# dmlc/difacto

Hardware: AMD Instinct MI355X
Metric: examples/sec (FM SGD worker step, Criteo-shape, V_dim=64) (higher is better)
Workload: dtype f32

## Files before the change

difacto_amd/capi.py:

```python
import ctypes as C
import os

import numpy as np

_HERE = os.path.dirname(os.path.abspath(__file__))
LIB_PATH = os.environ.get("DIFACTO_HIP_LIB") or os.path.join(_HERE, "libdifacto_hip.so")

FEA_COUNT, WEIGHT, GRADIENT = 1, 2, 3
INIT_REFRAND, INIT_HASH = 0, 1
U64MAX = 2 ** 64 - 1

SYMBOLS = [
    "dfh_last_error", "dfh_updater_param_default", "dfh_ctx_create", "dfh_ctx_destroy", "dfh_ctx_sync",
    "dfh_ctx_stream", "dfh_ctx_device", "dfh_reverse_bytes", "dfh_encode_fea_grp_id", "dfh_table_create",
    "dfh_table_destroy", "dfh_table_size", "dfh_table_param", "dfh_table_bytes", "dfh_pull", "dfh_push",
    "dfh_table_export", "dfh_table_import", "dfh_fm_predict", "dfh_fm_calcgrad", "dfh_loss_evaluate",
    "dfh_auc_times_n", "dfh_batch_create", "dfh_batch_destroy", "dfh_batch_load_host", "dfh_batch_load_device",
    "dfh_localize", "dfh_batch_load_localized_host", "dfh_batch_get_localized", "dfh_batch_shape", "dfh_sgd_step",
    "dfh_batch_progress", "dfh_batch_get_pred", "dfh_row_stride", "dfh_shard_pull", "dfh_shard_push_count",
    "dfh_shard_push_grad", "dfh_batch_forward", "dfh_batch_backward", "dfh_batch_device_keys", "dfh_malloc",
    "dfh_free", "dfh_memcpy_h2d", "dfh_memcpy_d2h", "dfh_ctx_set_timing", "dfh_ctx_get_timing", "dfh_kernel_name",
    "dfh_table_warm_start", "dfh_ctx_set_pipeline", "dfh_batch_lookup", "dfh_localize_lookup", "dfh_rowbuf_create", "dfh_rowbuf_destroy", "dfh_rowbuf_load_host", "dfh_batch_gather_rows", "dfh_batch_set_option", "dfh_batch_key_ranges", "dfh_batch_attach_device",
    "dfh_batch_key_ranges_device", "dfh_shard_resolve", "dfh_shard_pull_resolved", "dfh_shard_push_count_resolved",
    "dfh_shard_push_grad_resolved", "dfh_table_check", "dfh_ctx_set_timing_mask", "dfh_table_save", "dfh_table_load", "dfh_shard_resolve_multi", "dfh_shard_push_count_multi",
    "dfh_shard_push_grad_multi", "dfh_shard_count_pull_multi", "dfh_shard_push_grad_listed", "dfh_shard_release", "dfh_ctx_set_option", "dfh_table_set_has_aux", "dfh_table_has_aux",
    "dfh_comm_unique_id", "dfh_comm_create_rccl", "dfh_comm_create_callback", "dfh_comm_destroy", "dfh_comm_rank", "dfh_comm_world",
    "dfh_comm_allreduce_sum", "dfh_shard_create", "dfh_shard_destroy", "dfh_shard_owned_range", "dfh_shard_step", "dfh_shard_prefetch_counts",
    "dfh_shard_pull_host", "dfh_shard_push_host", "dfh_comm_allgather", "dfh_shard_balanced_splits", "dfh_shard_set_exchange", "dfh_shard_set_timing", "dfh_shard_get_timing",
    "dfh_comm_stats", "dfh_comm_info", "dfh_comm_selfcheck", "dfh_comm_wire_probe", "dfh_table_capacity", "dfh_batch_prepare_rows", "dfh_rowbuf_load_host_slices",
    "dfh_rowbuf_set_labels", "dfh_batch_prepare_cached", "dfh_batch_get_rows",
    "dfh_batch_create_many", "dfh_shard_multi_words", "dfh_shard_reserve", "dfh_comm_create_loopback", "dfh_comm_loopback_feed", "dfh_comm_loopback_wire", "dfh_comm_loopback_wire_time",
    "dfh_vec_inner_multi", "dfh_vec_combine", "dfh_vec_line_step", "dfh_lbfgs_create", "dfh_lbfgs_destroy", "dfh_lbfgs_add_chunk",
    "dfh_lbfgs_init_model", "dfh_lbfgs_shape", "dfh_lbfgs_get_model", "dfh_lbfgs_set_weights", "dfh_lbfgs_calc_grad",
    "dfh_lbfgs_prepare_direction", "dfh_lbfgs_calc_direction", "dfh_lbfgs_line_search", "dfh_lbfgs_evaluate", "dfh_lbfgs_create_sharded",
    "dfh_lbfgs_owned_range", "dfh_lbfgs_set_model", "dfh_bcd_set_model",
    "dfh_bcd_create", "dfh_bcd_destroy", "dfh_bcd_add_chunk", "dfh_bcd_build", "dfh_bcd_shape", "dfh_bcd_block_info",
    "dfh_bcd_epoch", "dfh_bcd_step", "dfh_bcd_get_model", "dfh_bcd_get_pred", "dfh_batch_split_entries",
    "dfh_bcd_create_sharded",
    "dfh_textchunk_create", "dfh_textchunk_destroy", "dfh_textchunk_parse_criteo", "dfh_textchunk_rows", "dfh_textchunk_ids",
    "dfh_rowbuf_load_slices",
]
XCHG_COUNTS, XCHG_KEYS, XCHG_CNT, XCHG_ROWS, XCHG_GRADS, XCHG_OTHER = range(6)
SHARD_STAGES = ("counts", "L", "K", "R", "RW", "F", "G", "P")
K_COUNT = 8
K_LOCALIZE, K_LOOKUP, K_FORWARD, K_BACKWARD, K_PULL, K_PUSH, K_MISC, K_AUC = range(8)


class UpdaterParam(C.Structure):
    _fields_ = [("l1", C.c_float), ("l2", C.c_float), ("V_l2", C.c_float), ("lr", C.c_float),
                ("lr_beta", C.c_float), ("V_lr", C.c_float), ("V_lr_beta", C.c_float),
                ("V_init_scale", C.c_float), ("V_dim", C.c_int), ("V_threshold", C.c_int),
                ("seed", C.c_uint), ("init_mode", C.c_int)]
# ... 30 lines not shown
            "%s is missing: build it with `python -m difacto_amd.build` (hipcc --offload-arch=gfx950). "
            "There is no CPU fallback." % LIB_PATH)
    if os.environ.get("DIFACTO_NO_TORCH_PRELOAD") != "1":
        try:
            import torch
        except ImportError:
            pass
    L = C.CDLL(LIB_PATH)
    vp, sz, i32, u64, f32 = C.c_void_p, C.c_size_t, C.c_int, C.c_uint64, C.c_float
    PP = C.POINTER
    L.dfh_last_error.restype = C.c_char_p
    L.dfh_updater_param_default.argtypes = [PP(UpdaterParam), i32]
    L.dfh_ctx_create.argtypes = [i32, vp, PP(vp)]
    L.dfh_ctx_destroy.argtypes = [vp]
    L.dfh_ctx_sync.argtypes = [vp]
    L.dfh_ctx_stream.restype = vp
    L.dfh_ctx_stream.argtypes = [vp]
    L.dfh_ctx_device.argtypes = [vp]
    L.dfh_reverse_bytes.restype = u64
    L.dfh_reverse_bytes.argtypes = [u64]
    L.dfh_encode_fea_grp_id.restype = u64
    L.dfh_encode_fea_grp_id.argtypes = [u64, i32, i32]
    L.dfh_table_create.argtypes = [vp, PP(UpdaterParam), u64, PP(vp)]
    L.dfh_table_destroy.argtypes = [vp]
    L.dfh_table_size.argtypes = [vp, PP(u64)]
    L.dfh_table_param.argtypes = [vp, PP(UpdaterParam)]
    L.dfh_table_capacity.argtypes = [vp, PP(u64), PP(u64)]
    L.dfh_table_bytes.restype = u64
    L.dfh_table_bytes.argtypes = [vp]
    L.dfh_pull.argtypes = [vp, vp, sz, vp, PP(sz), vp, PP(sz)]
    L.dfh_push.argtypes = [vp, vp, sz, i32, vp, sz, vp, sz]
    L.dfh_table_export.argtypes = [vp, u64, vp, vp, vp, vp, PP(u64)]
    L.dfh_table_import.argtypes = [vp, u64, vp, vp, vp, vp]
    L.dfh_fm_predict.argtypes = [vp, i32, sz, vp, vp, vp, vp, sz, vp, vp, sz, vp]
    L.dfh_fm_calcgrad.argtypes = [vp, i32, sz, vp, vp, vp, vp, vp, sz, vp, vp, sz, vp, vp]
    L.dfh_loss_evaluate.argtypes = [vp, vp, vp, sz, PP(f32)]
    L.dfh_auc_times_n.argtypes = [vp, vp, vp, sz, PP(f32)]
    L.dfh_batch_create.argtypes = [vp, sz, sz, PP(vp)]
    L.dfh_batch_destroy.argtypes = [vp]
    L.dfh_batch_create_many.argtypes = [vp, i32, sz, sz, PP(vp)]
    L.dfh_batch_split_entries.argtypes = [vp, vp]
    L.dfh_batch_load_host.argtypes = [vp, sz, vp, vp, vp, vp]
    L.dfh_batch_load_device.argtypes = [vp, sz, sz, vp, vp, vp, vp]
    L.dfh_batch_attach_device.argtypes = [vp, sz, sz, vp, vp, vp, vp]
    L.dfh_localize.argtypes = [vp, u64]
    L.dfh_batch_load_localized_host.argtypes = [vp, sz, vp, vp, vp, vp, vp, vp, sz]
    L.dfh_batch_get_localized.argtypes = [vp, PP(sz), vp, vp, vp]
    L.dfh_batch_shape.argtypes = [vp, PP(sz), PP(sz), PP(sz)]
    L.dfh_sgd_step.argtypes = [vp, vp, i32, i32]
    L.dfh_batch_progress.argtypes = [vp, PP(Progress), i32]
    L.dfh_batch_get_pred.argtypes = [vp, vp]
    L.dfh_row_stride.restype = sz
    L.dfh_row_stride.argtypes = [i32]
    L.dfh_shard_pull.argtypes = [vp, vp, sz, vp]
    L.dfh_shard_push_count.argtypes = [vp, vp, sz, vp]
    L.dfh_shard_push_grad.argtypes = [vp, vp, sz, vp]
# ... 147 lines not shown
class Context:

    def __init__(self, device=0, stream=None):
        self.h = C.c_void_p()
        _ck(lib().dfh_ctx_create(device, _dp(stream), C.byref(self.h)))

    def sync(self):
        _ck(lib().dfh_ctx_sync(self.h))

    def set_pipeline(self, on=True):
        _ck(lib().dfh_ctx_set_pipeline(self.h, int(on)))

    def set_option(self, name, value):
        _ck(lib().dfh_ctx_set_option(self.h, name.encode(), int(value)))

    def set_timing(self, on=True):
        _ck(lib().dfh_ctx_set_timing(self.h, 1 if on else 0))

    def set_timing_mask(self, mask):
        _ck(lib().dfh_ctx_set_timing_mask(self.h, mask))

    def get_timing(self, reset=True):
        ms = np.zeros(K_COUNT, np.float64)
        calls = np.zeros(K_COUNT, np.uint64)
        _ck(lib().dfh_ctx_get_timing(self.h, 1 if reset else 0, _p(ms), _p(calls)))
        return {lib().dfh_kernel_name(i).decode(): (float(ms[i]), int(calls[i])) for i in range(K_COUNT)}

    @property
    def stream(self):
        return lib().dfh_ctx_stream(self.h)
# ... 376 lines not shown
    def progress(self, reset=True):
        p = Progress()
        _ck(lib().dfh_batch_progress(self.h, C.byref(p), 1 if reset else 0))
        return p

    def pred(self):
        nrows, _, _ = self.shape(want_U=False)
        out = np.zeros(nrows, np.float32)
        _ck(lib().dfh_batch_get_pred(self.h, _p(out)))
        return out

    def split_entries(self):
        n = C.c_uint32(0)
        _ck(lib().dfh_batch_split_entries(self.h, C.byref(n)))
        return int(n.value)

    def forward(self, V_dim, d_rows):
        _ck(lib().dfh_batch_forward(self.h, V_dim, _dp(d_rows)))

    def backward(self, V_dim, d_rows, d_grads):
        _ck(lib().dfh_batch_backward(self.h, V_dim, _dp(d_rows), _dp(d_grads)))

    def key_ranges(self, nparts):
        out = np.zeros(nparts + 1, np.uint32)
        _ck(lib().dfh_batch_key_ranges(self.h, nparts, _p(out)))
        return out

    def device_keys(self):
        a, b, u = C.c_void_p(), C.c_void_p(), C.c_size_t(0)
        _ck(lib().dfh_batch_device_keys(self.h, C.byref(a), C.byref(b), C.byref(u)))
# ... 389 lines not shown
```

difacto_amd/csrc/dfh_api.hip:

```cpp
#include <algorithm>
#include <chrono>
#include <cstring>
#include <mutex>
#include <new>
#include <thread>

#include <hip/hip_ext.h>
#include <rocprim/rocprim.hpp>

#include "dfh_kernels.hip"
#include "dfh_localize.hip"
#include "dfh_update.hip"
#include "dfh_riders.hip"

using namespace dfh;

namespace dfh {
static thread_local std::string g_err;
void set_error(const std::string& msg) { g_err = msg; }
}

struct dfh_ctx {
  int device = 0;
  hipStream_t stream = nullptr;
  bool own_stream = false;
  std::vector<hipStream_t> preps;
  std::vector<hipStream_t> extra;
  hipStream_t parse = nullptr;
  std::mutex parse_mu;
  unsigned nprep = 0;
  unsigned next_prep = 0;
  bool pipeline = false;
  void* scratch = nullptr;
  size_t scratch_bytes = 0;
  int num_cu = 256;
  int fwd_depth = 5;
  int fwd_blocks = 0;
  int bwd_small_blocks = 2048;
  int upd_kernel = 1;
  int upd_hot_blocks = 512, upd_mid_blocks = 512, upd_few_blocks = 1024, upd_single_blocks = 4096;
  int upd_interleave = 0;
  int owner_per_key = 0;
  int upd_split = 1;
  int auc_in_update = 1;
  int shard_mixed_update = 1;
  int grow_initial_rows = 1 << 20;
  int event_flags = 1;
  int prep_priority = -1;
  int single_queue = 0;
  int rider_slot[4] = {2, 0, 1, 2};
  int rider_alone[4] = {0, 0, 0, 0};
  int rider_period[3] = {1, 1, 1};
  int rider_start[3] = {0, 0, 0};
  std::vector<dfh_batch*> pend;
  std::thread warm;
// ... 101 lines not shown
  uint32_t* d_split_ticket = nullptr;
  float* d_split_part = nullptr;
  size_t split_cap = 0;
  int split_sel = 0, split_last = 0;
  bool split_listing = false;
  uint32_t seg_nb = 0;
  uint2* d_uw = nullptr;
  uint32_t *d_urow = nullptr, *d_need = nullptr, *d_rank = nullptr, *d_total = nullptr;
  float *d_pred = nullptr, *d_slope = nullptr, *d_xv = nullptr;
  size_t xv_floats = 0;
  static constexpr size_t kProgDoubles = 2 * PROG_SLOTS + 64;
  double* d_prog = nullptr;
  float nrows_seen = 0;
  hipEvent_t ev_ready = nullptr, ev_free = nullptr;
  bool ready_pending = false, free_pending = false;
  hipStream_t prep = nullptr;
  bool compute_auc = false;
  uint32_t *d_auc_keys = nullptr, *d_auc_skeys = nullptr, *d_auc_lab = nullptr, *d_auc_slab = nullptr;
  uint32_t* d_auc_part = nullptr;
  uint32_t auc_pending_n = 0;
  bool force_radix = false;
  bool force_sort_fallback = false;
  dfh_table* looked_up = nullptr;
  struct GatherSeg { struct dfh_rowbuf* rb; size_t at, n; };
  std::vector<GatherSeg> gsegs;
  GatherSrc gsrc{};
  bool gather_pending = false, gather_fusable = false, gather_any_value = false, loc_fuse_gather = false;
  const uint32_t *g_rows = nullptr, *g_off = nullptr;
  const float* g_lab = nullptr;
  LocView loc_v{};
// ... 4 lines not shown
};

namespace dfh {
namespace chunks {
inline hipError_t reset_prog(dfh_batch* b, hipStream_t s);
}
}

namespace {
int flush_pending(dfh_batch* b);
void pend_remove(dfh_ctx* c, dfh_batch* b);
inline hipStream_t prep_of(const dfh_batch* b) {
  const dfh_ctx* c = b->ctx;
  return (c->pipeline && b->prep) ? b->prep : c->stream;
}
void phase_begin(dfh_batch* b) {
  dfh_ctx* c = b->ctx;
  if (b->pend_stage < RID_STAGES) (void)flush_pending(b);
  hipStream_t next = c->pipeline ? c->preps[c->next_prep++ % c->nprep] : nullptr;
  if (next && b->prep && next != b->prep && b->ready_pending) {
    (void)hipStreamWaitEvent(next, b->ev_ready, 0);
  }
  b->prep = next;
}
int prep_begin(dfh_batch* b) {
  dfh_ctx* c = b->ctx;
  if (c->pipeline && !b->prep) phase_begin(b);
  if (c->pipeline && b->free_pending) {
    DFH_HIP(hipStreamWaitEvent(prep_of(b), b->ev_free, 0));
    b->free_pending = false;
  }
  return DFH_OK;
}
int prep_end(dfh_batch* b) {
  dfh_ctx* c = b->ctx;
  if (c->pipeline && !b->defer_ready) {
    DFH_HIP(hipEventRecord(b->ev_ready, prep_of(b)));
    b->ready_pending = true;
  }
  return DFH_OK;
}
int main_begin(dfh_batch* b) {
  dfh_ctx* c = b->ctx;
  if (b->pend_stage < RID_STAGES) {
    int rc = flush_pending(b);
    if (rc) return rc;
  }
  if (b->ready_pending) {
    DFH_HIP(hipStreamWaitEvent(c->stream, b->ev_ready, 0));
    b->ready_pending = false;
  }
  return DFH_OK;
}
int main_end(dfh_batch* b) {
  dfh_ctx* c = b->ctx;
  if (b->split_listing) {
    b->split_listing = false;
    b->split_last = b->split_sel;
    b->split_sel ^= 1;
  }
  if (c->pipeline) {
    DFH_HIP(hipEventRecord(b->ev_free, c->stream));
    b->free_pending = true;
  }
  return DFH_OK;
}
int sync_all(dfh_ctx* c) {
  for (hipStream_t p : c->preps) DFH_HIP(hipStreamSynchronize(p));
  for (hipStream_t p : c->extra) DFH_HIP(hipStreamSynchronize(p));
  DFH_HIP(hipStreamSynchronize(c->stream));
  return DFH_OK;
}
inline bool split_listed(const dfh_ctx* c, const dfh_batch* b, int is_train) { return b && is_train && c->upd_kernel && c->upd_split; }
inline uint32_t* split_counter(const dfh_batch* b) { return b->d_U + 2 + b->split_sel; }
inline SplitOut split_out(const dfh_ctx* c, dfh_batch* b, int is_train, uint32_t u_base) {
  if (!split_listed(c, b, is_train)) return SplitOut{nullptr, nullptr, 0u, 0u};
  b->split_listing = true;
  return SplitOut{b->d_split_ent, split_counter(b), u_base, (uint32_t)b->split_cap};
}
}

namespace {

inline int grid_for_threads(size_t n, const dfh_ctx* c) {
  size_t b = (n + 255) / 256;
  size_t cap = (size_t)c->num_cu * 8;
  return (int)std::max<size_t>(1, std::min(b, cap));
}
inline int grid_for_waves(size_t nwaves, const dfh_ctx* c) {
  size_t b = (nwaves + 3) / 4;
  size_t cap = (size_t)c->num_cu * 8;
  return (int)std::max<size_t>(1, std::min(b, cap));
}

int ensure_scratch(dfh_ctx* c, size_t bytes) {
  if (bytes <= c->scratch_bytes) return DFH_OK;
  if (c->scratch) {
    DFH_HIP(hipStreamSynchronize(c->stream));
    DFH_HIP(hipFree(c->scratch));
    c->scratch = nullptr;
    c->scratch_bytes = 0;
  }
// ... 491 lines not shown

inline int count_mode(const dfh_ctx* c, int is_train, int push_cnt) { return push_cnt ? ((is_train && c->upd_kernel) ? 2 : 1) : 0; }

struct StepExtras {
  uint32_t* need = nullptr;
  bool pre = false;
  bool riders = false;
  bool spans = false;
};

int step_lookup(dfh_table* t, dfh_batch* b, int is_train, int push_cnt, uint32_t lo, const uint32_t* d_n, size_t n, const StepExtras& x,
                const float* rrows = nullptr, size_t U = 0, hipEvent_t rows_in = nullptr) {
  dfh_ctx* c = t->ctx;
  hipStream_t s = c->stream;
  const float* cnt = b->has_cnt ? b->d_feacnt + lo : (const float*)nullptr;
  const int mode = count_mode(c, is_train, push_cnt), gl = grid_for_threads(n, c);
  const uint32_t n_static = d_n ? 0u : (uint32_t)n;
  static const bool gap_trace = getenv("DFH_GAP_TRACE") != nullptr;
  const bool ride = x.spans && gap_trace && ((c->timing >> DFH_K_LOOKUP) & 1u);
  TimeScope ts(c, (x.spans && !ride) ? DFH_K_LOOKUP : DFH_K_COUNT);
  const SplitOut so = split_out(c, b, is_train, lo);
  RiderSet rs;
  rs.n = 0;
  if (x.riders) collect_riders(c, 0, true, ((uint32_t)gl + 7u) / 8u, &rs);
  if (rrows) {
    DFH_HIP(hipStreamWaitEvent(s, rows_in, 0));
    const UwRemote m{rrows, dfh_row_stride(t->v.k), b->d_U, lo, lo + (uint32_t)n, b->d_uw, b->d_col_ptr, split_out(c, b, is_train, 0u), t->v.err};
    hipLaunchKernelGGL(k_lookup_uw_remote, dim3(grid_for_threads(U, c)), dim3(256), 0, s, t->v, b->d_feaids + lo, n_static, b->d_urow + lo,
                       cnt, b->d_col_ptr + lo, mode, b->d_uw + lo, auc_pending(b), m, so);
  } else if (rs.n) {
    hipLaunchKernelGGL(k_lookup_riders, dim3((((unsigned)gl + 7u) / 8u + rs.ngroups) * 8u), dim3(256), rider_smem(rs), s, t->v,
                       b->d_feaids + lo, d_n, n_static, b->d_urow + lo, cnt, b->d_col_ptr + lo, mode, x.need, x.pre ? 1 : 0, b->d_uw + lo,
                       auc_pending(b), so, (uint32_t)gl, rs);
  } else {
    launch_span(c, ride, DFH_K_LOOKUP, 1, k_lookup_step, dim3(gl), dim3(256), 0, s, t->v, b->d_feaids + lo, d_n, n_static, b->d_urow + lo,
                cnt, b->d_col_ptr + lo, mode, x.need, x.pre ? 1 : 0, b->d_uw + lo, auc_pending(b), so);
  }
  b->auc_pending_n = 0;
  DFH_HIP(hipGetLastError());
  return DFH_OK;
}

struct StepRemote {
// ... 193 lines not shown
  } else if (n == "grow_initial_rows") {
    DFH_ARG(value >= 16 && value <= (1 << 28), "grow_initial_rows must be in [16, 2^28]");
    c->grow_initial_rows = value;
  } else if (n == "auc_in_update") {
    DFH_ARG(value == 0 || value == 1, "auc_in_update must be 0 (k_auc_pairs as its own launch) or 1 (a role of k_update_fused)");
    c->auc_in_update = value;
  } else if (n == "shard_mixed_update") {
    DFH_ARG(value == 0 || value == 1, "shard_mixed_update must be 0 or 1");
    c->shard_mixed_update = value;
  } else if (n == "owner_per_key") {
    DFH_ARG(value == 0 || value == 1, "owner_per_key must be 0 (count push, Pull, gradient push per received entry) or 1 (per distinct key)");
    c->owner_per_key = value;
  } else if (n == "upd_split") {
    DFH_ARG(value == 0 || value == 1, "upd_split must be 0 (one block per hot key, whatever its length) or 1 (a block per part of 1 024 occurrences)");
    c->upd_split = value;
  } else if (n == "upd_interleave") {
    DFH_ARG(value >= 0 && value <= 64, "upd_interleave must be in [0, 64]");
    c->upd_interleave = value;
  } else if (n == "event_flags") {
    DFH_ARG(value == 0 || value == 1, "event_flags must be 0 (default events) or 1 (no system-scope fence); set before batches are created");
    c->event_flags = value;
  } else if (n == "single_queue") {
    DFH_ARG(value == 0 || value == 1, "single_queue must be 0 (preparation streams) or 1 (the Localizer's stages ride in the step's launches)");
    if (value != c->single_queue) {
      for (dfh_batch* p : std::vector<dfh_batch*>(c->pend)) {
        int rcf = flush_pending(p);
        if (rcf) return rcf;
      }
      int rcs = sync_all(c);
      if (rcs) return rcs;
// ... 11 lines not shown
    c->rider_alone[st] = (value >> 2) & 1;
  } else if (n == "rider_start_lookup" || n == "rider_start_forward" || n == "rider_start_update") {
    DFH_ARG(value >= 0 && value <= 100, "rider_start_*: per cent of the carrier's own blocks dispatched before the first rider group");
    c->rider_start[n == "rider_start_lookup" ? 0 : n == "rider_start_forward" ? 1 : 2] = value;
  } else if (n == "rider_period_lookup" || n == "rider_period_forward" || n == "rider_period_update") {
    DFH_ARG(value >= 1 && value <= 4096, "rider_period_*: one group of 8 rider blocks every n groups (1: riders first)");
    c->rider_period[n == "rider_period_lookup" ? 0 : n == "rider_period_forward" ? 1 : 2] = value;
  } else if (n == "prep_priority") {
    DFH_ARG(value >= -1 && value <= 1, "prep_priority must be -1 (lowest), 0 (default) or 1 (highest)");
    DFH_ARG(c->preps.empty(), "prep_priority must be set before dfh_ctx_set_pipeline creates the streams");
    c->prep_priority = value;
  } else {
    set_error("dfh_ctx_set_option: unknown option " + n);
    return DFH_ERR_ARG;
  }
  return DFH_OK;
}
void* dfh_ctx_stream(dfh_ctx* c) { return c ? c->stream : nullptr; }
int dfh_ctx_device(dfh_ctx* c) { return c ? c->device : -1; }

int dfh_ctx_set_timing(dfh_ctx* c, int enable) {
  DFH_ARG(c, "ctx is NULL");
  c->timing = enable ? ~0u : 0u;
  return DFH_OK;
}

int dfh_ctx_set_timing_mask(dfh_ctx* c, uint32_t mask) {
  DFH_ARG(c, "ctx is NULL");
  c->timing = mask;
  return DFH_OK;
// ... 1419 lines not shown
  } else {
    hipLaunchKernelGGL(k_rdx_keys, dim3(g), dim3(256), 0, s, b->d_raw, N, max_index, b->d_keys, b->d_pos);
    size_t tb = b->temp_bytes;
    DFH_HIP(rocprim::radix_sort_pairs(b->d_temp, tb, b->d_keys, b->d_skeys, b->d_pos, b->d_spos, (size_t)N, 0, 64, s));
    hipLaunchKernelGGL(k_rdx_heads, dim3(g), dim3(256), 0, s, b->d_skeys, N, b->d_head);
    tb = b->temp_bytes;
    DFH_HIP(rocprim::inclusive_scan(b->d_temp, tb, b->d_head, b->d_uid, (size_t)N, rocprim::plus<uint32_t>(), s));
    hipLaunchKernelGGL(k_rdx_emit, dim3(g), dim3(256), 0, s, b->d_skeys, b->d_spos, b->d_head, b->d_uid, N, (uint32_t)b->nrows,
                       b->d_offset, b->has_value ? b->d_value : (const float*)nullptr, b->d_feaids, b->d_col_ptr, b->d_index,
                       b->d_s_row, b->d_s_val, b->d_U);
    hipLaunchKernelGGL(k_seg_lists_reset, dim3(1), dim3(64), 0, s, b->d_mid, b->d_hot, b->d_few, b->d_U + 2);
    hipLaunchKernelGGL(k_seg_lists, dim3((unsigned)std::max<size_t>(1, std::min<size_t>((N + 1023) / 1024, 256))), dim3(1024), 0, s,
                       b->d_col_ptr, b->d_U, b->d_mid, b->d_hot, b->d_few, b->d_mid_ent, b->d_hot_ent, b->d_few_ent);
    b->seg_nb = 1;
    if (probe)
      hipLaunchKernelGGL(k_lookup, dim3(grid_for_threads(b->nnz, c)), dim3(256), 0, s, probe->v, b->d_feaids, b->d_U, 0u, b->d_urow,
                         (const float*)nullptr, b->d_col_ptr, 0, (uint32_t*)nullptr, 0, (uint2*)nullptr, AucFin{nullptr, 0u, nullptr});
  }
  delete tsp;
  DFH_HIP(hipGetLastError());
  b->localized = true;
  b->has_cnt = false;
  if (probe) b->looked_up = probe;
  return prep_end(b);
}
}


int dfh_localize(dfh_batch* b, uint64_t max_index) {
  DFH_ARG(b && b->nrows > 0, "dfh_localize: no batch loaded");
  DFH_ARG(max_index != 0, "max_index must be nonzero");
// ... 35 lines not shown
    set_error("dfh_batch_lookup: batch is not localized");
    return DFH_ERR_STATE;
  }
  dfh_ctx* c = b->ctx;
  if (b->nnz == 0) return DFH_OK;
  if (b->nnz <= kSmallBatchPairs) return DFH_OK;
  if (c->single_queue) return DFH_OK;
  DFH_HIP(hipSetDevice(c->device));
  int rc = table_reserve(t, b->nnz);
  if (rc) return rc;
  rc = prep_begin(b);
  if (rc) return rc;
  {
    hipStream_t ps = prep_of(b);
    TimeScope ts(c, DFH_K_LOOKUP, ps);
    hipLaunchKernelGGL(k_lookup, dim3(grid_for_threads(b->nnz, c)), dim3(256), 0, ps, t->v, b->d_feaids, b->d_U, 0u,
                       b->d_urow, (const float*)nullptr, b->d_col_ptr, 0, (uint32_t*)nullptr, 0, (uint2*)nullptr, AucFin{nullptr, 0u, nullptr});
  }
  DFH_HIP(hipGetLastError());
  b->looked_up = t;
  return prep_end(b);
}

int dfh_batch_load_localized_host(dfh_batch* b, size_t nrows, const size_t* offset, const uint32_t* index, const float* value,
                                  const float* label, const uint64_t* feaids, const float* feacnt, size_t U) {
  DFH_ARG(b && offset && label && feaids, "dfh_batch_load_localized_host: NULL argument");
  DFH_ARG(nrows >= 1 && nrows <= b->max_rows, "nrows out of range");
  std::vector<uint32_t> off32;
  int rc = to_u32_offsets(offset, nrows, &off32);
  if (rc) return rc;
  const size_t base = offset[0], nnz = off32[nrows];
// ... 196 lines not shown
  if (is_train && refrand) {
    rc = refrand_flush(t, b->d_feaids, b->d_U, Nb, b->d_urow, b->d_need, b->d_rank, b->d_total);
    if (rc) return rc;
  }
  return main_end(b);
}

int dfh_batch_split_entries(dfh_batch* b, uint32_t* n) {
  DFH_ARG(b && n, "dfh_batch_split_entries: NULL argument");
  dfh_ctx* c = b->ctx;
  DFH_HIP(hipSetDevice(c->device));
  if (b->pend_stage < RID_STAGES) {
    int rc = flush_pending(b);
    if (rc) return rc;
  }
  if (b->ready_pending) DFH_HIP(hipStreamWaitEvent(c->stream, b->ev_ready, 0));
  DFH_HIP(hipMemcpyAsync(n, b->d_U + 2 + b->split_last, sizeof(uint32_t), hipMemcpyDeviceToHost, c->stream));
  DFH_HIP(hipStreamSynchronize(c->stream));
  return DFH_OK;
}

int dfh_batch_forward(dfh_batch* b, int V_dim, const float* d_rows) {
  DFH_ARG(b && b->localized && d_rows, "dfh_batch_forward: bad argument");
  const int kp = (V_dim + 3) / 4 * 4;
  int rc = ensure_xv(b, kp);
  if (rc) return rc;
  b->nrows_seen += (float)b->nrows;
  rc = main_begin(b);
  if (rc) return rc;
  rc = launch_forward(b, packed_src(d_rows, V_dim), V_dim, kp);
  if (rc) return rc;
  return main_end(b);
}
// ... 99 lines not shown
```

difacto_amd/csrc/dfh_feed.hip:

```cpp
struct dfh_rowbuf {
  dfh_ctx* ctx = nullptr;
  size_t max_rows = 0, max_nnz = 0, nrows = 0, nnz = 0;
  uint32_t* d_off = nullptr;
  uint64_t* d_idx = nullptr;
  float* d_val = nullptr;
  float* d_lab = nullptr;
  bool has_value = false, has_labels = false;
  hipStream_t up = nullptr;
  hipEvent_t ev_loaded = nullptr;
  struct Used { hipStream_t stream; hipEvent_t ev; bool pending; };
  std::mutex mu;
  std::vector<Used> used;
  std::vector<hipStream_t> seen_loaded;
  double t_prof[3] = {0, 0, 0};
  uint64_t n_prof = 0, bytes_prof = 0;
  std::vector<uint32_t> off32;
};

namespace {
int localize_impl(dfh_batch* b, uint64_t max_index, dfh_table* probe);

struct PrepLaps {
  double* acc;
  bool on;
// ... 303 lines not shown
  gs.dst_off = b->d_offset;
  gs.dst_lab = b->d_label;
  batch_loaded(b, nrows, in.nnz, in.any_value);
  return DFH_OK;
}

int queue_described(dfh_table* t, dfh_batch* b, const DescribedIn& in, uint64_t max_index, PrepLaps& laps) {
  dfh_ctx* c = b->ctx;
  int rc = describe(b, in);
  if (rc) return rc;
  laps.lap(3);
  b->defer_ready = true;
  rc = localize_impl(b, max_index, nullptr);
  laps.lap(4);
  if (!rc && in.nnz > kSmallBatchPairs && !c->single_queue) {
    hipLaunchKernelGGL(k_lookup, dim3(grid_for_threads(b->nnz, c)), dim3(256), 0, prep_of(b), t->v, b->d_feaids, b->d_U, 0u, b->d_urow,
                       (const float*)nullptr, b->d_col_ptr, 0, (uint32_t*)nullptr, 0, (uint2*)nullptr, AucFin{nullptr, 0u, nullptr});
    if (hipGetLastError() != hipSuccess) rc = DFH_ERR_HIP;
    b->looked_up = t;
  }
  b->defer_ready = false;
  if (rc) return rc;
  rc = prep_end(b);
  laps.lap(5);
  if (laps.on) ++b->n_prof;
  return rc;
}
}

extern "C" {

// ... 224 lines not shown
```

difacto_amd/csrc/dfh_kernels.hip:

```cpp
#include "dfh_internal.h"

namespace dfh {

__device__ __forceinline__ int lane_id() { return threadIdx.x & 63; }

__device__ __forceinline__ float wave_sum(float v) {
#pragma unroll
  for (int o = 32; o > 0; o >>= 1) v += __shfl_xor(v, o, 64);
  return v;
}

template <int L>
__device__ __forceinline__ float cross_group_sum(float v) {
#pragma unroll
  for (int o = L; o < 64; o <<= 1) v += __shfl_xor(v, o, 64);
  return v;
}
template <int L>
__device__ __forceinline__ float in_group_sum(float v) {
#pragma unroll
  for (int o = L >> 1; o > 0; o >>= 1) v += __shfl_xor(v, o, 64);
  return v;
}

// ... 378 lines not shown
  uint32_t u_base;
  uint32_t cap;
};
__device__ __forceinline__ uint32_t* split_other(uint32_t* n) { return reinterpret_cast<uint32_t*>(reinterpret_cast<uintptr_t>(n) ^ 4u); }
__device__ __forceinline__ void lookup_split(const SplitOut& so, uint32_t* err, uint32_t u, uint32_t beg, uint32_t end) {
  if (!(DFH_HOT_SPLIT_BUILD & 1) || !so.ent || end - beg <= HOT_SPLIT_MIN) return;
  const uint32_t nparts = (end - beg + HOT_SPLIT - 1u) / HOT_SPLIT;
  const uint32_t base = atomicAdd(so.n, nparts);
  if (base + nparts > so.cap) {
    atomicOr(err, 16u);
    return;
  }
  for (uint32_t p = 0; p < nparts; ++p)
    so.ent[base + p] = make_uint4(u + so.u_base, beg + p * HOT_SPLIT, min(beg + (p + 1u) * HOT_SPLIT, end), (p << 16) | nparts);
}

template <bool SPLIT = true>
__device__ __forceinline__ void lookup_body(const TableView& t, const uint64_t* __restrict__ keys, const uint32_t* __restrict__ d_n,
                         uint32_t n_static, uint32_t* __restrict__ urow, const float* __restrict__ cnt,
                         const uint32_t* __restrict__ col_ptr, int push_cnt, uint32_t* __restrict__ need_init,
                         int rows_known, uint2* __restrict__ uw, AucFin fin, const uint32_t bid, const uint32_t nblk,
                         const SplitOut so = SplitOut{nullptr, nullptr, 0u, 0u}) {
  if (fin.n && bid == 0) auc_finalize_block(fin);
  if (SPLIT && so.n && bid == 0 && threadIdx.x == 0) *split_other(so.n) = 0u;
  uint32_t n = d_n ? *d_n : n_static;
  __shared__ uint32_t ins_sh[8];
  for (uint32_t u0 = bid * blockDim.x; u0 < n; u0 += nblk * blockDim.x) {
    const uint32_t u = u0 + threadIdx.x;
    const bool active = u < n;
    uint64_t key = active ? keys[u] : 0ull;
// ... 1781 lines not shown
```

difacto_amd/csrc/dfh_shard.hip:

```cpp
#ifndef DFH_SHARD_HIP_
#define DFH_SHARD_HIP_
#include <dlfcn.h>
#include <link.h>

#include <chrono>
#include <deque>
#include <optional>
#include <thread>

namespace dfh {

struct RcclId { char internal[128]; };
struct RcclApi {
  void* lib = nullptr;
  int (*GetUniqueId)(RcclId*) = nullptr;
  int (*CommInitRank)(void**, int, RcclId, int) = nullptr;
  int (*CommDestroy)(void*) = nullptr;
  const char* (*GetErrorString)(int) = nullptr;
  int (*Send)(const void*, size_t, int, int, void*, hipStream_t) = nullptr;
  int (*Recv)(void*, size_t, int, int, void*, hipStream_t) = nullptr;
  int (*GroupStart)() = nullptr;
  int (*GroupEnd)() = nullptr;
  int (*GetVersion)(int*) = nullptr;
  std::string path;
// ... 1066 lines not shown
int shard_step_overlap(dfh_shard* s, dfh_batch* b, int is_train, int push_cnt, int* any_active) {
  dfh_comm* c = s->c;
  dfh_ctx* ctx = s->t->ctx;
  DFH_HIP(hipSetDevice(ctx->device));
  hipStream_t st = ctx->stream, cs = s->cs;
  int rc;
  if (s->timing) ++s->stage_steps;
  static const bool trace = getenv("DFH_SHARD_TRACE") != nullptr;
  Flight& cur = s->fl[s->cur];
  if (trace)
    fprintf(stderr, "[shard %d] step %llu: b=%p cur{slot %d described %d pulled %d b=%p} armed %d next_b=%p\n", c->rank,
            (unsigned long long)s->steps, (void*)b, s->cur, (int)cur.described, (int)cur.pulled, (void*)cur.b, (int)s->next_armed,
            (void*)s->next_b);
  if (!(cur.described && cur.b == b)) {
    DFH_ARG(!cur.described || !cur.pulled, "dfh_shard_step: the batch differs from the one announced to dfh_shard_prefetch_counts");
    if (b && b->ready_pending) DFH_HIP(hipStreamWaitEvent(cs, b->ev_ready, 0));
    {
      StageScope ts(s, DFH_SHARD_STAGE_COUNTS, cs);
      rc = queue_counts(s, b, cs);
      if (rc) return rc;
    }
    DFH_HIP(hipStreamSynchronize(cs));
    flight_sizes(s, cur, b, s->cur);
  }
  if (any_active) *any_active = cur.active != 0 ? 1 : 0;
  ++s->steps;
  if (b) b->nrows_seen += (float)b->nrows;
  const bool look = s->next_armed;
  dfh_batch* nb = look ? s->next_b : nullptr;
  s->next_armed = false;
  Flight& nxt = s->fl[s->cur ^ 1];
  nxt = Flight();
  if (cur.active == 0) {
    cur = Flight();
    return b ? main_end(b) : DFH_OK;
  }
  auto keys_out = [&](Flight& f) {
    const int q = f.slot;
    hipEvent_t ready = f.b && f.b->ready_pending ? f.b->ev_ready : nullptr;
    hipEvent_t freed = s->p_pending[q] ? s->ev_p[q] : nullptr;
    s->p_pending[q] = false;
    return flight_K(s, f, push_cnt, cs, ready, freed, s->ev_k[q]);
  };
  auto rows_back = [&](Flight& f) {
    const int q = f.slot;
    int r = flight_R(s, f, push_cnt, s->ev_k[q], s->ev_r[q]);
    if (!r) r = flight_RW(s, f, cs, s->ev_r[q], s->ev_rw[q]);
    f.pulled = r == DFH_OK;
    return r;
  };
  rc = flight_bufs(s, cur);
  if (rc) return rc;
  if (b) {
    rc = main_begin(b);
    if (rc) return rc;
  }
  const int q = cur.slot;
  const bool uw_folded = cur.any_own && cur.pulled && cur.any_remote && b != nullptr;
  if ((rc = flight_L(s, cur, is_train, push_cnt, uw_folded ? s->ev_rw[q] : nullptr))) return rc;
  if (!cur.pulled) {
    if ((rc = keys_out(cur)) || (rc = rows_back(cur))) return rc;
  }
  if (look) {
    if (nb && nb->ready_pending) DFH_HIP(hipStreamWaitEvent(cs, nb->ev_ready, 0));
    StageScope ts(s, DFH_SHARD_STAGE_COUNTS, cs);
    rc = queue_counts(s, nb, cs);
    if (rc) return rc;
    DFH_HIP(hipEventRecord(s->cnt_ev, cs));
  }
  if ((rc = flight_F(s, cur, is_train, push_cnt, uw_folded, uw_folded ? nullptr : s->ev_rw[q], s->ev_f))) return rc;
  bool ahead = false;
  if (look) {
    DFH_HIP(hipEventSynchronize(s->cnt_ev));
    flight_sizes(s, nxt, nb, s->cur ^ 1);
    ahead = nxt.active != 0;
    if (trace)
      fprintf(stderr, "[shard %d]   next: active %zu U %zu nrecv %zu own [%u, %u) -> ahead %d\n", c->rank, nxt.active, nxt.U, nxt.nrecv,
              nxt.own_lo, nxt.own_hi, (int)ahead);
    if (ahead) {
// ... 318 lines not shown
```

include/difacto_hip.h:

```cpp
#ifndef DIFACTO_HIP_H_
#define DIFACTO_HIP_H_
#include <stddef.h>
#include <stdint.h>

#ifdef __cplusplus
extern "C" {
#endif

enum {
  DFH_OK = 0,
  DFH_ERR_ARG = 1,
  DFH_ERR_HIP = 2,
  DFH_ERR_CAPACITY = 3,
  DFH_ERR_STATE = 4
};

enum { DFH_FEA_COUNT = 1, DFH_WEIGHT = 2, DFH_GRADIENT = 3 };

enum {
  DFH_INIT_REFRAND = 0,
  DFH_INIT_HASH = 1
};

typedef struct {
// ... 13 lines not shown
typedef struct dfh_ctx dfh_ctx;
typedef struct dfh_table dfh_table;
typedef struct dfh_batch dfh_batch;

const char* dfh_last_error(void);
void dfh_updater_param_default(dfh_updater_param* p, int V_dim);

int dfh_ctx_create(int device, void* stream, dfh_ctx** out);
int dfh_ctx_destroy(dfh_ctx* ctx);
int dfh_ctx_sync(dfh_ctx* ctx);
void* dfh_ctx_stream(dfh_ctx* ctx);
int dfh_ctx_device(dfh_ctx* ctx);

int dfh_ctx_set_pipeline(dfh_ctx* ctx, int enable);
int dfh_ctx_set_option(dfh_ctx* ctx, const char* name, int value);

enum {
  DFH_K_LOCALIZE = 0, DFH_K_LOOKUP, DFH_K_FORWARD, DFH_K_BACKWARD, DFH_K_PULL, DFH_K_PUSH, DFH_K_MISC, DFH_K_AUC, DFH_K_COUNT
};
int dfh_ctx_set_timing(dfh_ctx* ctx, int enable);
int dfh_ctx_set_timing_mask(dfh_ctx* ctx, uint32_t mask);
int dfh_ctx_get_timing(dfh_ctx* ctx, int reset, double* total_ms, uint64_t* calls);
const char* dfh_kernel_name(int id);

uint64_t dfh_reverse_bytes(uint64_t x);
uint64_t dfh_encode_fea_grp_id(uint64_t x, int gid, int nbits);

int dfh_table_create(dfh_ctx* ctx, const dfh_updater_param* p, uint64_t capacity_rows, dfh_table** out);
int dfh_table_capacity(dfh_table* t, uint64_t* capacity_rows, uint64_t* grows);
int dfh_table_destroy(dfh_table* t);
// ... 72 lines not shown
int dfh_rowbuf_set_labels(dfh_rowbuf* rb, size_t nrows, const float* label);
int dfh_batch_prepare_cached(dfh_table* t, dfh_batch* b, size_t nrows, int nseg, dfh_rowbuf* const* bufs, const uint32_t* const* rows,
                             const size_t* seg_rows, uint64_t max_index);

int dfh_batch_load_localized_host(dfh_batch* b, size_t nrows, const size_t* offset, const uint32_t* index,
                                  const float* value, const float* label, const uint64_t* feaids,
                                  const float* feacnt, size_t U);
int dfh_batch_get_localized(dfh_batch* b, size_t* U, uint64_t* feaids, float* feacnt, uint32_t* index);
int dfh_batch_shape(dfh_batch* b, size_t* nrows, size_t* nnz, size_t* U);
int dfh_batch_get_rows(dfh_batch* b, uint32_t* offset, float* label);

int dfh_sgd_step(dfh_table* t, dfh_batch* b, int is_train, int push_cnt);
int dfh_batch_progress(dfh_batch* b, dfh_progress* out, int reset);
int dfh_batch_get_pred(dfh_batch* b, float* pred);
int dfh_batch_split_entries(dfh_batch* b, uint32_t* n);

size_t dfh_row_stride(int V_dim);
int dfh_shard_pull(dfh_table* t, const uint64_t* d_keys, size_t n, float* d_rows);
int dfh_shard_push_count(dfh_table* t, const uint64_t* d_keys, size_t n, const float* d_cnt);
int dfh_shard_push_grad(dfh_table* t, const uint64_t* d_keys, size_t n, const float* d_grads);
int dfh_batch_forward(dfh_batch* b, int V_dim, const float* d_rows);
int dfh_batch_backward(dfh_batch* b, int V_dim, const float* d_rows, float* d_grads);
int dfh_batch_device_keys(dfh_batch* b, const uint64_t** d_feaids, const float** d_feacnt, size_t* U);
int dfh_batch_key_ranges(dfh_batch* b, int nparts, uint32_t* bounds);
int dfh_batch_key_ranges_device(dfh_batch* b, int nparts, const uint64_t* d_splits, int64_t* d_bounds);

int dfh_shard_resolve(dfh_table* t, const uint64_t* d_keys, size_t n, uint32_t* d_rowid);
int dfh_shard_pull_resolved(dfh_table* t, const uint32_t* d_rowid, size_t n, float* d_rows);
int dfh_shard_push_count_resolved(dfh_table* t, const uint32_t* d_rowid, const uint64_t* d_keys, size_t n, const float* d_cnt);
int dfh_shard_push_grad_resolved(dfh_table* t, const uint32_t* d_rowid, const uint64_t* d_keys, size_t n, const float* d_grads);
// ... 104 lines not shown
```

Before: 88.40 million.

## Defer batch ready-event records and shrink lookup grid to K keys per thread

Batch readiness events are no longer recorded at the end of each prep phase. They are owed and recorded lazily, only when a consumer needs them or before more work is queued on the same prep stream, which cuts the number of hipEventRecord calls. Separately, lookup kernels now launch a grid sized for DFH_LOOKUP_K (default 2) slots per thread, with an optional lookup_blocks override. The launch sizing assumes the lookup kernel body grid-strides over the extra slots. Deferred recording adds bookkeeping and could misorder events if a flush point is missed.

Result: slower. 86.55 million (-2.1%).

```diff
diff --git a/difacto_amd/capi.py b/difacto_amd/capi.py
--- a/difacto_amd/capi.py
+++ b/difacto_amd/capi.py
@@ -36,6 +36,7 @@
     "dfh_lbfgs_owned_range", "dfh_lbfgs_set_model", "dfh_bcd_set_model",
     "dfh_bcd_create", "dfh_bcd_destroy", "dfh_bcd_add_chunk", "dfh_bcd_build", "dfh_bcd_shape", "dfh_bcd_block_info",
     "dfh_bcd_epoch", "dfh_bcd_step", "dfh_bcd_get_model", "dfh_bcd_get_pred", "dfh_batch_split_entries",
+    "dfh_batch_get_lookup", "dfh_ctx_ready_records",
     "dfh_bcd_create_sharded",
     "dfh_textchunk_create", "dfh_textchunk_destroy", "dfh_textchunk_parse_criteo", "dfh_textchunk_rows", "dfh_textchunk_ids",
     "dfh_rowbuf_load_slices",
@@ -96,6 +97,7 @@
     L.dfh_ctx_create.argtypes = [i32, vp, PP(vp)]
     L.dfh_ctx_destroy.argtypes = [vp]
     L.dfh_ctx_sync.argtypes = [vp]
+    L.dfh_ctx_ready_records.argtypes = [vp, PP(u64)]
     L.dfh_ctx_stream.restype = vp
     L.dfh_ctx_stream.argtypes = [vp]
     L.dfh_ctx_device.argtypes = [vp]
@@ -122,6 +124,7 @@
     L.dfh_batch_destroy.argtypes = [vp]
     L.dfh_batch_create_many.argtypes = [vp, i32, sz, sz, PP(vp)]
     L.dfh_batch_split_entries.argtypes = [vp, vp]
+    L.dfh_batch_get_lookup.argtypes = [vp, vp, vp]
     L.dfh_batch_load_host.argtypes = [vp, sz, vp, vp, vp, vp]
     L.dfh_batch_load_device.argtypes = [vp, sz, sz, vp, vp, vp, vp]
     L.dfh_batch_attach_device.argtypes = [vp, sz, sz, vp, vp, vp, vp]
@@ -299,6 +302,11 @@
     def set_option(self, name, value):
         _ck(lib().dfh_ctx_set_option(self.h, name.encode(), int(value)))
 
+    def ready_records(self):
+        n = C.c_uint64(0)
+        _ck(lib().dfh_ctx_ready_records(self.h, C.byref(n)))
+        return int(n.value)
+
     def set_timing(self, on=True):
         _ck(lib().dfh_ctx_set_timing(self.h, 1 if on else 0))
 
@@ -705,6 +713,13 @@
         n = C.c_uint32(0)
         _ck(lib().dfh_batch_split_entries(self.h, C.byref(n)))
         return int(n.value)
+
+    def get_lookup(self):
+        _, _, U = self.shape()
+        urow = np.zeros(max(U, 1), np.uint32)
+        uw = np.zeros((max(U, 1), 2), np.uint32)
+        _ck(lib().dfh_batch_get_lookup(self.h, _p(urow), _p(uw)))
+        return urow[:U], uw[:U]
 
     def forward(self, V_dim, d_rows):
         _ck(lib().dfh_batch_forward(self.h, V_dim, _dp(d_rows)))
diff --git a/difacto_amd/csrc/dfh_api.hip b/difacto_amd/csrc/dfh_api.hip
--- a/difacto_amd/csrc/dfh_api.hip
+++ b/difacto_amd/csrc/dfh_api.hip
@@ -28,6 +28,8 @@
   std::vector<hipStream_t> extra;
   hipStream_t parse = nullptr;
   std::mutex parse_mu;
+  std::vector<dfh_batch*> owing;
+  uint64_t ready_records = 0;
   unsigned nprep = 0;
   unsigned next_prep = 0;
   bool pipeline = false;
@@ -39,6 +41,7 @@
   int bwd_small_blocks = 2048;
   int upd_kernel = 1;
   int upd_hot_blocks = 512, upd_mid_blocks = 512, upd_few_blocks = 1024, upd_single_blocks = 4096;
+  int lookup_blocks = 0;
   int upd_interleave = 0;
   int owner_per_key = 0;
   int upd_split = 1;
@@ -170,6 +173,8 @@
   float nrows_seen = 0;
   hipEvent_t ev_ready = nullptr, ev_free = nullptr;
   bool ready_pending = false, free_pending = false;
+  bool ready_owed = false;
+  hipStream_t owed_on = nullptr;
   hipStream_t prep = nullptr;
   bool compute_auc = false;
   uint32_t *d_auc_keys = nullptr, *d_auc_skeys = nullptr, *d_auc_lab = nullptr, *d_auc_slab = nullptr;
@@ -204,8 +209,30 @@
   const dfh_ctx* c = b->ctx;
   return (c->pipeline && b->prep) ? b->prep : c->stream;
 }
+int ready_flush(dfh_batch* b) {
+  if (!b->ready_owed) return DFH_OK;
+  dfh_ctx* c = b->ctx;
+  b->ready_owed = false;
+  c->owing.erase(std::remove(c->owing.begin(), c->owing.end(), b), c->owing.end());
+  DFH_HIP(hipEventRecord(b->ev_ready, b->owed_on));
+  ++c->ready_records;
+  return DFH_OK;
+}
+int ready_flush_stream(dfh_ctx* c, hipStream_t s, const dfh_batch* except, bool all = false) {
+  for (dfh_batch* o : std::vector<dfh_batch*>(c->owing))
+    if (o != except && (all || o->owed_on == s)) {
+      int rc = ready_flush(o);
+      if (rc) return rc;
+    }
+  return DFH_OK;
+}
+inline hipEvent_t ready_event(dfh_batch* b) {
+  if (!b || !b->ready_pending) return nullptr;
+  return ready_flush(b) == DFH_OK ? b->ev_ready : nullptr;
+}
 void phase_begin(dfh_batch* b) {
   dfh_ctx* c = b->ctx;
+  (void)ready_flush(b);
   if (b->pend_stage < RID_STAGES) (void)flush_pending(b);
   hipStream_t next = c->pipeline ? c->preps[c->next_prep++ % c->nprep] : nullptr;
   if (next && b->prep && next != b->prep && b->ready_pending) {
@@ -216,6 +243,10 @@
 int prep_begin(dfh_batch* b) {
   dfh_ctx* c = b->ctx;
   if (c->pipeline && !b->prep) phase_begin(b);
+  if (c->pipeline) {
+    int rc = ready_flush_stream(c, prep_of(b), b);
+    if (rc) return rc;
+  }
   if (c->pipeline && b->free_pending) {
     DFH_HIP(hipStreamWaitEvent(prep_of(b), b->ev_free, 0));
     b->free_pending = false;
@@ -225,7 +256,13 @@
 int prep_end(dfh_batch* b) {
   dfh_ctx* c = b->ctx;
   if (c->pipeline && !b->defer_ready) {
-    DFH_HIP(hipEventRecord(b->ev_ready, prep_of(b)));
+    if (b->ready_owed && b->owed_on != prep_of(b)) {
+      int rc = ready_flush(b);
+      if (rc) return rc;
+    }
+    if (!b->ready_owed) c->owing.push_back(b);
+    b->ready_owed = true;
+    b->owed_on = prep_of(b);
     b->ready_pending = true;
   }
   return DFH_OK;
@@ -234,6 +271,10 @@
   dfh_ctx* c = b->ctx;
   if (b->pend_stage < RID_STAGES) {
     int rc = flush_pending(b);
+    if (rc) return rc;
+  }
+  {
+    int rc = ready_flush_stream(c, nullptr, nullptr, true);
     if (rc) return rc;
   }
   if (b->ready_pending) {
@@ -256,6 +297,10 @@
   return DFH_OK;
 }
 int sync_all(dfh_ctx* c) {
+  {
+    int rc = ready_flush_stream(c, nullptr, nullptr, true);
+    if (rc) return rc;
+  }
   for (hipStream_t p : c->preps) DFH_HIP(hipStreamSynchronize(p));
   for (hipStream_t p : c->extra) DFH_HIP(hipStreamSynchronize(p));
   DFH_HIP(hipStreamSynchronize(c->stream));
@@ -276,6 +321,10 @@
   size_t b = (n + 255) / 256;
   size_t cap = (size_t)c->num_cu * 8;
   return (int)std::max<size_t>(1, std::min(b, cap));
+}
+inline int lookup_grid(size_t n, const dfh_ctx* c, bool exact = false) {
+  if (c->lookup_blocks) return c->lookup_blocks;
+  return grid_for_threads(exact ? n : (n + DFH_LOOKUP_K - 1) / DFH_LOOKUP_K, c);
 }
 inline int grid_for_waves(size_t nwaves, const dfh_ctx* c) {
   size_t b = (nwaves + 3) / 4;
@@ -797,7 +846,7 @@
   dfh_ctx* c = t->ctx;
   hipStream_t s = c->stream;
   const float* cnt = b->has_cnt ? b->d_feacnt + lo : (const float*)nullptr;
-  const int mode = count_mode(c, is_train, push_cnt), gl = grid_for_threads(n, c);
+  const int mode = count_mode(c, is_train, push_cnt), gl = lookup_grid(n, c, d_n == nullptr);
   const uint32_t n_static = d_n ? 0u : (uint32_t)n;
   static const bool gap_trace = getenv("DFH_GAP_TRACE") != nullptr;
   const bool ride = x.spans && gap_trace && ((c->timing >> DFH_K_LOOKUP) & 1u);
@@ -809,7 +858,7 @@
   if (rrows) {
     DFH_HIP(hipStreamWaitEvent(s, rows_in, 0));
     const UwRemote m{rrows, dfh_row_stride(t->v.k), b->d_U, lo, lo + (uint32_t)n, b->d_uw, b->d_col_ptr, split_out(c, b, is_train, 0u), t->v.err};
-    hipLaunchKernelGGL(k_lookup_uw_remote, dim3(grid_for_threads(U, c)), dim3(256), 0, s, t->v, b->d_feaids + lo, n_static, b->d_urow + lo,
+    hipLaunchKernelGGL(k_lookup_uw_remote, dim3(lookup_grid(U, c, true)), dim3(256), 0, s, t->v, b->d_feaids + lo, n_static, b->d_urow + lo,
                        cnt, b->d_col_ptr + lo, mode, b->d_uw + lo, auc_pending(b), m, so);
   } else if (rs.n) {
     hipLaunchKernelGGL(k_lookup_riders, dim3((((unsigned)gl + 7u) / 8u + rs.ngroups) * 8u), dim3(256), rider_smem(rs), s, t->v,
@@ -1033,6 +1082,9 @@
   } else if (n == "upd_split") {
     DFH_ARG(value == 0 || value == 1, "upd_split must be 0 (one block per hot key, whatever its length) or 1 (a block per part of 1 024 occurrences)");
     c->upd_split = value;
+  } else if (n == "lookup_blocks") {
+    DFH_ARG(value >= 0 && value <= 65536, "lookup_blocks must be in [0, 65536] (0: automatic, one trip over nnz slots)");
+    c->lookup_blocks = value;
   } else if (n == "upd_interleave") {
     DFH_ARG(value >= 0 && value <= 64, "upd_interleave must be in [0, 64]");
     c->upd_interleave = value;
@@ -1074,6 +1126,11 @@
     set_error("dfh_ctx_set_option: unknown option " + n);
     return DFH_ERR_ARG;
   }
+  return DFH_OK;
+}
+int dfh_ctx_ready_records(dfh_ctx* c, uint64_t* n) {
+  DFH_ARG(c && n, "dfh_ctx_ready_records: NULL argument");
+  *n = c->ready_records;
   return DFH_OK;
 }
 void* dfh_ctx_stream(dfh_ctx* c) { return c ? c->stream : nullptr; }
@@ -2523,7 +2580,7 @@
                        b->d_col_ptr, b->d_U, b->d_mid, b->d_hot, b->d_few, b->d_mid_ent, b->d_hot_ent, b->d_few_ent);
     b->seg_nb = 1;
     if (probe)
-      hipLaunchKernelGGL(k_lookup, dim3(grid_for_threads(b->nnz, c)), dim3(256), 0, s, probe->v, b->d_feaids, b->d_U, 0u, b->d_urow,
+      hipLaunchKernelGGL(k_lookup, dim3(lookup_grid(b->nnz, c)), dim3(256), 0, s, probe->v, b->d_feaids, b->d_U, 0u, b->d_urow,
                          (const float*)nullptr, b->d_col_ptr, 0, (uint32_t*)nullptr, 0, (uint2*)nullptr, AucFin{nullptr, 0u, nullptr});
   }
   delete tsp;
@@ -2589,7 +2646,7 @@
   {
     hipStream_t ps = prep_of(b);
     TimeScope ts(c, DFH_K_LOOKUP, ps);
-    hipLaunchKernelGGL(k_lookup, dim3(grid_for_threads(b->nnz, c)), dim3(256), 0, ps, t->v, b->d_feaids, b->d_U, 0u,
+    hipLaunchKernelGGL(k_lookup, dim3(lookup_grid(b->nnz, c)), dim3(256), 0, ps, t->v, b->d_feaids, b->d_U, 0u,
                        b->d_urow, (const float*)nullptr, b->d_col_ptr, 0, (uint32_t*)nullptr, 0, (uint2*)nullptr, AucFin{nullptr, 0u, nullptr});
   }
   DFH_HIP(hipGetLastError());
@@ -2816,9 +2873,22 @@
     int rc = flush_pending(b);
     if (rc) return rc;
   }
-  if (b->ready_pending) DFH_HIP(hipStreamWaitEvent(c->stream, b->ev_ready, 0));
+  if (hipEvent_t e = ready_event(b)) DFH_HIP(hipStreamWaitEvent(c->stream, e, 0));
   DFH_HIP(hipMemcpyAsync(n, b->d_U + 2 + b->split_last, sizeof(uint32_t), hipMemcpyDeviceToHost, c->stream));
   DFH_HIP(hipStreamSynchronize(c->stream));
+  return DFH_OK;
+}
+
+int dfh_batch_get_lookup(dfh_batch* b, uint32_t* urow, uint32_t* uw) {
+  DFH_ARG(b && b->localized && (urow || uw), "dfh_batch_get_lookup: bad argument");
+  dfh_ctx* c = b->ctx;
+  DFH_HIP(hipSetDevice(c->device));
+  int rc = sync_all(c);
+  if (rc) return rc;
+  uint32_t U = 0;
+  DFH_HIP(hipMemcpy(&U, b->d_U, sizeof(uint32_t), hipMemcpyDeviceToHost));
+  if (urow && U) DFH_HIP(hipMemcpy(urow, b->d_urow, (size_t)U * sizeof(uint32_t), hipMemcpyDeviceToHost));
+  if (uw && U) DFH_HIP(hipMemcpy(uw, b->d_uw, (size_t)U * sizeof(uint2), hipMemcpyDeviceToHost));
   return DFH_OK;
 }
 
diff --git a/difacto_amd/csrc/dfh_feed.hip b/difacto_amd/csrc/dfh_feed.hip
--- a/difacto_amd/csrc/dfh_feed.hip
+++ b/difacto_amd/csrc/dfh_feed.hip
@@ -341,7 +341,7 @@
   rc = localize_impl(b, max_index, nullptr);
   laps.lap(4);
   if (!rc && in.nnz > kSmallBatchPairs && !c->single_queue) {
-    hipLaunchKernelGGL(k_lookup, dim3(grid_for_threads(b->nnz, c)), dim3(256), 0, prep_of(b), t->v, b->d_feaids, b->d_U, 0u, b->d_urow,
+    hipLaunchKernelGGL(k_lookup, dim3(lookup_grid(b->nnz, c)), dim3(256), 0, prep_of(b), t->v, b->d_feaids, b->d_U, 0u, b->d_urow,
                        (const float*)nullptr, b->d_col_ptr, 0, (uint32_t*)nullptr, 0, (uint2*)nullptr, AucFin{nullptr, 0u, nullptr});
     if (hipGetLastError() != hipSuccess) rc = DFH_ERR_HIP;
     b->looked_up = t;
diff --git a/difacto_amd/csrc/dfh_kernels.hip b/difacto_amd/csrc/dfh_kernels.hip
--- a/difacto_amd/csrc/dfh_kernels.hip
+++ b/difacto_amd/csrc/dfh_kernels.hip
@@ -416,6 +416,10 @@
   for (uint32_t p = 0; p < nparts; ++p)
     so.ent[base + p] = make_uint4(u + so.u_base, beg + p * HOT_SPLIT, min(beg + (p + 1u) * HOT_SPLIT, end), (p << 16) | nparts);
 }
+
+#ifndef DFH_LOOKUP_K
+#define DFH_LOOKUP_K 2
+#endif
 
 template <bool SPLIT = true>
 __device__ __forceinline__ void lookup_body(const TableView& t, const uint64_t* __restrict__ keys, const uint32_t* __restrict__ d_n,
diff --git a/difacto_amd/csrc/dfh_shard.hip b/difacto_amd/csrc/dfh_shard.hip
--- a/difacto_amd/csrc/dfh_shard.hip
+++ b/difacto_amd/csrc/dfh_shard.hip
@@ -1104,7 +1104,7 @@
             (void*)s->next_b);
   if (!(cur.described && cur.b == b)) {
     DFH_ARG(!cur.described || !cur.pulled, "dfh_shard_step: the batch differs from the one announced to dfh_shard_prefetch_counts");
-    if (b && b->ready_pending) DFH_HIP(hipStreamWaitEvent(cs, b->ev_ready, 0));
+    if (hipEvent_t e = ready_event(b)) DFH_HIP(hipStreamWaitEvent(cs, e, 0));
     {
       StageScope ts(s, DFH_SHARD_STAGE_COUNTS, cs);
       rc = queue_counts(s, b, cs);
@@ -1127,7 +1127,7 @@
   }
   auto keys_out = [&](Flight& f) {
     const int q = f.slot;
-    hipEvent_t ready = f.b && f.b->ready_pending ? f.b->ev_ready : nullptr;
+    hipEvent_t ready = ready_event(f.b);
     hipEvent_t freed = s->p_pending[q] ? s->ev_p[q] : nullptr;
     s->p_pending[q] = false;
     return flight_K(s, f, push_cnt, cs, ready, freed, s->ev_k[q]);
@@ -1152,7 +1152,7 @@
     if ((rc = keys_out(cur)) || (rc = rows_back(cur))) return rc;
   }
   if (look) {
-    if (nb && nb->ready_pending) DFH_HIP(hipStreamWaitEvent(cs, nb->ev_ready, 0));
+    if (hipEvent_t e = ready_event(nb)) DFH_HIP(hipStreamWaitEvent(cs, e, 0));
     StageScope ts(s, DFH_SHARD_STAGE_COUNTS, cs);
     rc = queue_counts(s, nb, cs);
     if (rc) return rc;
diff --git a/include/difacto_hip.h b/include/difacto_hip.h
--- a/include/difacto_hip.h
+++ b/include/difacto_hip.h
@@ -51,6 +51,7 @@
 
 int dfh_ctx_set_pipeline(dfh_ctx* ctx, int enable);
 int dfh_ctx_set_option(dfh_ctx* ctx, const char* name, int value);
+int dfh_ctx_ready_records(dfh_ctx* ctx, uint64_t* n);
 
 enum {
   DFH_K_LOCALIZE = 0, DFH_K_LOOKUP, DFH_K_FORWARD, DFH_K_BACKWARD, DFH_K_PULL, DFH_K_PUSH, DFH_K_MISC, DFH_K_AUC, DFH_K_COUNT
@@ -153,6 +154,7 @@
 int dfh_batch_progress(dfh_batch* b, dfh_progress* out, int reset);
 int dfh_batch_get_pred(dfh_batch* b, float* pred);
 int dfh_batch_split_entries(dfh_batch* b, uint32_t* n);
+int dfh_batch_get_lookup(dfh_batch* b, uint32_t* urow, uint32_t* uw);
 
 size_t dfh_row_stride(int V_dim);
 int dfh_shard_pull(dfh_table* t, const uint64_t* d_keys, size_t n, float* d_rows);
```
